# sunshinnnn/DSMnet

Measured on AMD Instinct MI355X. Metric: stereo pairs/sec forward, PSMNet D=192 384×1280, at 1/2/4/8 MI355X, higher is better.
Workload: dtype f32

## Files before the change

dsmnet_amd/csrc/deconv_zs.hpp:

```cpp
#pragma once


template <int PM> struct DzsCfg {
  static constexpr int NP = Prec<PM>::NP, NPW = Prec<PM>::NPW;
  static constexpr int THREADS = 512, NSTAGE = 256;
  static constexpr int TY = 2, IY = TY + 1, IX = 33;
  static constexpr int NV = IY * IX;
  static constexpr int NPF = (NV * 8 + NSTAGE - 1) / NSTAGE;
  static constexpr int NVP = 32 * NPF;
  static constexpr int ROW = NVP * 16;
  static constexpr int IMG = NP * 4 * ROW;
  static constexpr int XPL = 2 * TY * 64 * 8 * 16;
  static constexpr int LDS = 2 * IMG + 2 * XPL;
  static constexpr int NSTEP = 27;
#ifndef DSM_DZS_DEPTH
#define DSM_DZS_DEPTH 4
#endif
  static constexpr int DEPTH = DSM_DZS_DEPTH;
  static_assert(DEPTH == 2 || DEPTH == 4, "the staging loop is unrolled four times");
  static constexpr int WRING = 9, WAHEAD = 8;
  static_assert(NSTEP % WRING == 0 && WAHEAD < WRING, "weight ring");
  static_assert(LDS <= 160 * 1024, "LDS");
};

template <int PM>
__global__ __launch_bounds__(512, 1) void deconv_zs_kernel(ConvParams p) {
  using C = DzsCfg<PM>;
  using T = ZsTerms<PM>;
  using frag = typename Prec<PM>::frag;
  constexpr int NP = C::NP, NPW = C::NPW, TY = C::TY, IX = C::IX, NV = C::NV, NPF = C::NPF, ROW = C::ROW,
                IMG = C::IMG, XPL = C::XPL, NSTEP = C::NSTEP, WRING = C::WRING, WAHEAD = C::WAHEAD;
  extern __shared__ __attribute__((aligned(16))) unsigned char lds_raw[];
  const int tid = threadIdx.x, lane = tid & 63, wave = tid >> 6;
  const bool staging = wave >= 4;
  const int w4 = wave & 3;
  const int ncg = p.Cin >> 5;
  const int NTP = p.Cout >> 5;
  const int MD = (p.Do + 1) >> 1;

  const int G = gridDim.x, id = blockIdx.x;
  const int logical = (G & 7) == 0 ? (id & 7) * (G >> 3) + (id >> 3) : id;
  const long nunits = (long)p.ntiles * MD;
  const long u_begin = nunits * logical / G, u_end = nunits * (logical + 1) / G;
  if (u_begin >= u_end) return;

  const SplitScale ss = split_scale<PM>(p.x_amax, p.w_amax);
  const float sx = ss.sx, so = ss.out;
  unsigned char* const xch = lds_raw + 2 * IMG;
  float am = 0.f;

  struct It { long u; int col, m0, m1, zhi, zi, cg; bool valid; };
  auto open_segment = [&](long u) {
    It q; q.u = u; q.valid = u < u_end;
    if (!q.valid) { q.col = q.m0 = q.m1 = q.zhi = q.zi = q.cg = 0; return q; }
    q.col = (int)(u / MD); q.m0 = (int)(u % MD);
    q.m1 = (int)min((long)MD, (long)q.m0 + (u_end - u));
    q.zhi = 2 * q.m1 - 1 < p.Do ? q.m1 : q.m1 - 1;
    q.zi = q.m0; q.cg = 0;
    return q;
  };
  auto advance = [&](It q) {
    if (++q.cg < ncg) return q;
    q.cg = 0;
    if (++q.zi <= q.zhi) return q;
    return open_segment(q.u + (q.m1 - q.m0));
  };
  auto handover = [&](const It& q) {
    if (!q.valid || q.cg != ncg - 1) return 0u;
    unsigned m = 0;
    if (q.zi - 1 >= q.m0 && q.zi - 1 < q.m1 && 2 * q.zi - 1 < p.Do) m |= 1u;
    if (q.zi >= q.m0 && q.zi < q.m1) m |= 2u;
    return m;
  };

  if (staging) {
    const int stid = tid & 255;
    const unsigned vstride = (unsigned)p.Cin * 4u;
    const unsigned plane_bytes = vstride * (unsigned)p.Hi * (unsigned)p.Wi;
    constexpr unsigned OOBV = 0x80000000u;
    const int sq = 2 * (lane >> 4) + (lane & 1), sv = 8 * w4 + ((lane & 15) >> 1);
    unsigned voff[NPF];
    auto column_offsets = [&](int col) {
      const int t = col / NTP;
      const int y0 = ((t / p.ntx) % p.nty) * TY, x0 = (t % p.ntx) * 32;
#pragma unroll
      for (int k = 0; k < NPF; ++k) {
        const int v = sv + 32 * k;
        const int y = y0 + v / IX, x = x0 + v % IX;
        const bool ok = v < NV && y < p.Hi && x < p.Wi;
        voff[k] = ok ? ((unsigned)y * (unsigned)p.Wi + (unsigned)x) * vstride + 16u * (unsigned)sq : OOBV;
      }
    };
    f32x4 pf[C::DEPTH][NPF];
    auto load_chunk = [&](auto setc, const It& q) {
      constexpr int set = decltype(setc)::value;
      const int b = (q.col / NTP) / (p.ntx * p.nty);
      const bool live = q.valid && q.zi < p.Di;
      const long off = live ? ((long)b * p.Di + q.zi) * (long)plane_bytes + (long)q.cg * 128 : 0;
      const __amdgpu_buffer_rsrc_t rs = make_rsrc(reinterpret_cast<const char*>(p.x) + off, live ? plane_bytes : 0u);
#pragma unroll
      for (int k = 0; k < NPF; ++k) pf[set][k] = buffer_load16(rs, voff[k], 0);
    };
    const int st_off = (lane >> 4) * ROW + sv * 16 + (lane & 1) * 8;
    auto split_chunk = [&](auto setc, unsigned char* wr) {
      constexpr int set = decltype(setc)::value;
#pragma unroll
      for (int k = 0; k < NPF; ++k) {
        unsigned lo[NP], hi[NP];
        split_pair<PM>(pf[set][k].x, pf[set][k].y, sx, lo);
        split_pair<PM>(pf[set][k].z, pf[set][k].w, sx, hi);
#pragma unroll
        for (int q = 0; q < NP; ++q) {
          u32x2 v; v.x = lo[q]; v.y = hi[q];
          *reinterpret_cast<u32x2*>(wr + q * 4 * ROW + 512 * k) = v;
        }
      }
    };
    const int qd = stid & 7, ev = stid >> 3;
    f32x4 sc[2], sh[2];
#pragma unroll
    for (int nb = 0; nb < 2; ++nb) {
      const int c = 32 * (nb < NTP ? nb : 0) + 4 * qd;
#pragma unroll
      for (int e = 0; e < 4; ++e) {
        sc[nb][e] = p.scale ? p.scale[c + e] * so : so;
        sh[nb][e] = p.shift ? p.shift[c + e] : 0.f;
      }
    }
    struct Pend { int col, zi; unsigned m; };
    struct Where { int b, Y0, X0, nb; };
    auto where = [&](int col) {
      Where q;
      const int t = col / NTP;
      q.nb = col - t * NTP;
      q.b = t / (p.ntx * p.nty);
      q.Y0 = 2 * (((t / p.ntx) % p.nty) * TY);
      q.X0 = 2 * ((t % p.ntx) * 32);
      return q;
    };
    f32x4 resq[2][8];
#pragma unroll
    for (int s = 0; s < 2; ++s)
#pragma unroll
      for (int k = 0; k < 8; ++k) resq[s][k] = f32x4{0.f, 0.f, 0.f, 0.f};
    auto vmask_of = [&](const Where& q) {
      unsigned m = 0;
#pragma unroll
      for (int k = 0; k < 8; ++k)
        if (q.Y0 + (k >> 1) < p.Ho && q.X0 + ev + 32 * (k & 1) < p.Wo) m |= 1u << k;
      return m;
    };
    auto load_res = [&](const Pend& e) __attribute__((always_inline)) {
      if (!e.m || !p.res) return;
      const Where q = where(e.col);
      const unsigned vm = vmask_of(q);
#pragma unroll
      for (int s = 0; s < 2; ++s) {
        if (!((e.m >> s) & 1u)) continue;
        const float* const rb = p.res + ((((long)q.b * p.Dr + 2 * e.zi - 1 + s) * p.Hr + q.Y0) * p.Wr + q.X0 + ev) * p.Cout +
                                32 * q.nb + 4 * qd;
#pragma unroll
        for (int k = 0; k < 8; ++k)
          if ((vm >> k) & 1u)
            resq[s][k] = *reinterpret_cast<const f32x4*>(rb + ((k >> 1) * p.Wr + 32 * (k & 1)) * p.Cout);
      }
    };
    const float lo2 = p.relu == 2 ? 0.f : -__builtin_huge_valf(), lo1 = p.relu == 1 ? 0.f : -__builtin_huge_valf();
    auto vmax = [](f32x4 v, float lo) {
      v.x = fmaxf(v.x, lo); v.y = fmaxf(v.y, lo); v.z = fmaxf(v.z, lo); v.w = fmaxf(v.w, lo);
      return v;
    };
    auto epilogue = [&](const Pend& e) __attribute__((always_inline)) {
      if (!e.m) return;
      const Where q = where(e.col);
      const unsigned vm = vmask_of(q);
      const f32x4 s_ = q.nb ? sc[1] : sc[0], h_ = q.nb ? sh[1] : sh[0];
#pragma unroll
      for (int s = 0; s < 2; ++s) {
        if (!((e.m >> s) & 1u)) continue;
        f32x4 v[8];
#pragma unroll
        for (int k = 0; k < 8; ++k) {
          const int oy = k >> 1, ox = ev + 32 * (k & 1);
          v[k] = *reinterpret_cast<const f32x4*>(xch + s * XPL + ((oy * 64 + ox) * 8 + (qd ^ ((ox >> 1) & 7))) * 16);
        }
        float* const yb = p.y + ((((long)q.b * p.Do + 2 * e.zi - 1 + s) * p.Ho + q.Y0) * p.Wo + q.X0 + ev) * p.Cout +
                          32 * q.nb + 4 * qd;
#pragma unroll
        for (int k = 0; k < 8; ++k) {
          if (!((vm >> k) & 1u)) continue;
          f32x4 o = vmax(v[k] * s_ + h_, lo2);
          if (p.res) o += resq[s][k];
          o = vmax(o, lo1);
          *reinterpret_cast<f32x4*>(yb + ((k >> 1) * p.Wo + 32 * (k & 1)) * p.Cout) = o;
          track_amax(am, o);
        }
      }
    };

    constexpr int D = C::DEPTH;
    It c0 = open_segment(u_begin);
    It lead = c0;
    column_offsets(c0.col);
    load_chunk(std::integral_constant<int, 0>{}, lead);
    split_chunk(std::integral_constant<int, 0>{}, lds_raw + st_off);
    static_for<1, D>([&](auto dc) {
      const It nl = advance(lead);
      if (nl.valid && nl.col != lead.col) column_offsets(nl.col);
      lead = nl;
      load_chunk(dc, lead);
    });
    It c1 = advance(c0);
    Pend pend = {0, 0, 0u};
    load_res(Pend{c0.col, c0.zi, handover(c0)});
    __syncthreads();
    auto iteration = [&](auto pc) {
      constexpr int P = decltype(pc)::value;
      const It nl = advance(lead);
      if (nl.valid && nl.col != lead.col) column_offsets(nl.col);
      lead = nl;
      load_chunk(std::integral_constant<int, P % D>{}, lead);
      if (c1.valid) split_chunk(std::integral_constant<int, (P + 1) % D>{}, lds_raw + ((P + 1) & 1) * IMG + st_off);
      epilogue(pend);
      pend = Pend{c0.col, c0.zi, handover(c0)};
      load_res(Pend{c1.col, c1.zi, handover(c1)});
      __syncthreads();
      c0 = c1; c1 = advance(c1);
      return !c0.valid;
    };
    while (true) {
      if (iteration(std::integral_constant<int, 0>{})) break;
      if (iteration(std::integral_constant<int, 1>{})) break;
      if (iteration(std::integral_constant<int, 2>{})) break;
      if (iteration(std::integral_constant<int, 3>{})) break;
    }
    epilogue(pend);
  } else {
    const int j = lane & 15, kg = lane >> 4;
    const int ah = w4 >> 1, xh = w4 & 1;
    const unsigned tstride = (unsigned)NTP * (NPW * 1024);
    const __amdgpu_buffer_rsrc_t wrsrc = make_rsrc(p.w, p.wbytes);
    const unsigned wlane = (unsigned)(kg >> 1) * 27u * tstride + (unsigned)(32 * (kg & 1) + 16 * ah + j) * 16u;
    auto wbase_of = [&](const It& q) {
      return (unsigned)q.cg * 54u * tstride + (unsigned)(q.col % NTP) * (NPW * 1024);
    };
    const int rd_off = kg * ROW + (16 * xh + j) * 16;
    f32x4 acc[3][4][TY];
    frag xq[2][TY][NP];
    frag wq[WRING][NP];
    auto zero_set = [&](auto sc_) {
      constexpr int s = decltype(sc_)::value;
#pragma unroll
      for (int c = 0; c < 4; ++c)
#pragma unroll
        for (int r = 0; r < TY; ++r) acc[s][c][r] = f32x4{0.f, 0.f, 0.f, 0.f};
    };
    auto wload = [&](auto sc_, unsigned wb) {
      constexpr int s = decltype(sc_)::value;
      constexpr int tap = (s % 3) * 9 + dc_tap9(s / 3);
#pragma unroll
      for (int q = 0; q < NP; ++q)
        wq[s % WRING][q] = __builtin_bit_cast(frag, buffer_load16(wrsrc, wlane, wb + (unsigned)tap * tstride + q * 1024));
    };
    auto xload = [&](auto oc, const unsigned char* rd) {
      constexpr int o = decltype(oc)::value, iy = o >> 1, ix = o & 1;
#pragma unroll
      for (int r = 0; r < TY; ++r)
#pragma unroll
        for (int q = 0; q < NP; ++q)
          xq[o & 1][r][q] = *reinterpret_cast<const frag*>(rd + q * 4 * ROW + ((r + iy) * IX + ix) * 16);
    };
    auto zmask_of = [&](const It& q) {
      unsigned m = 0;
      if (q.zi >= q.m0 && q.zi < q.m1) m |= 6u;
      if (q.zi - 1 >= q.m0 && q.zi - 1 < q.m1 && q.zi < p.Di && 2 * q.zi - 1 < p.Do) m |= 1u;
      return m;
    };
    It cur = open_segment(u_begin);
    static_for<0, 3>([&](auto s) { zero_set(s); });
    static_for<0, WAHEAD>([&](auto sc_) { wload(sc_, wbase_of(cur)); });
    int i = 0;
    __syncthreads();
    while (true) {
      const unsigned char* const rd = lds_raw + (i & 1) * IMG + rd_off;
      const It nxt = advance(cur);
      const unsigned wcur = wbase_of(cur);
      const unsigned wnext = nxt.valid ? wbase_of(nxt) : 0u;
      const unsigned mask = zmask_of(cur);
      xload(std::integral_constant<int, 0>{}, rd);
      __builtin_amdgcn_sched_barrier(0);
      static_for<0, NSTEP>([&](auto sc_) {
        constexpr int s = decltype(sc_)::value;
        constexpr int jp = s / 3, kz = s % 3;
        constexpr DcPair pr = dc_pair(jp);
        constexpr bool fresh = kz == 0 && (jp == 0 || jp == 4 || jp == 6 || jp == 8);
        if constexpr (s + WAHEAD < NSTEP) wload(std::integral_constant<int, s + WAHEAD>{}, wcur);
        else wload(std::integral_constant<int, s + WAHEAD - NSTEP>{}, wnext);
        if constexpr (fresh && pr.o + 1 < 4) xload(std::integral_constant<int, pr.o + 1>{}, rd);
        __builtin_amdgcn_sched_barrier(0);
        if ((mask >> kz) & 1u) {
          static_for<0, T::N>([&](auto tc) {
            constexpr int t = decltype(tc)::value;
            static_for<0, TY>([&](auto rc) {
              constexpr int r = decltype(rc)::value;
              acc[kz][pr.c][r] = zs_mfma<PM>(wq[s % WRING][T::w[t]], xq[pr.o & 1][r][T::x[t]], acc[kz][pr.c][r]);
            });
          });
        }
        __builtin_amdgcn_sched_barrier(0);
      });
      if (cur.cg == ncg - 1) {
        const unsigned m = handover(cur);
#pragma unroll
        for (int s = 0; s < 2; ++s) {
          if (!((m >> s) & 1u)) continue;
#pragma unroll
          for (int c = 0; c < 4; ++c)
#pragma unroll
            for (int r = 0; r < TY; ++r) {
              const int oy = 2 * r + (c >> 1), ox = 2 * (16 * xh + j) + (c & 1);
              const int unit = (oy * 64 + ox) * 8 + ((4 * ah + kg) ^ (j & 7));
              *reinterpret_cast<f32x4*>(xch + s * XPL + unit * 16) = acc[s][c][r];
            }
        }
#pragma unroll
        for (int c = 0; c < 4; ++c)
#pragma unroll
          for (int r = 0; r < TY; ++r) acc[0][c][r] = acc[2][c][r];
        zero_set(std::integral_constant<int, 1>{});
        zero_set(std::integral_constant<int, 2>{});
      }
      __syncthreads();
      cur = nxt; ++i;
      if (!cur.valid) break;
    }
  }
  publish_amax<8>(p.y_amax, am, reinterpret_cast<float*>(lds_raw));
}

template <int PM>
int run_deconv_zs(ConvParams p, hipStream_t s) {
  using C = DzsCfg<PM>;
  DSM_REQUIRE(p.Cin % 64 == 0 && (p.Cout == 32 || p.Cout == 64) && 4l * p.Hi * p.Wi * p.Cin < 0x7fffffffl,
              DSM_ERR_UNSUPPORTED);
  p.ntx = dsm_cdiv(p.Wi, 32); p.nty = dsm_cdiv(p.Hi, C::TY);
  const long ncol = (long)p.B * p.nty * p.ntx * (p.Cout / 32);
  DSM_REQUIRE(ncol * p.Di < (1L << 30), DSM_ERR_UNSUPPORTED);
  p.ntiles = (int)ncol;
  const long nunits = ncol * ((p.Do + 1) / 2);
  DSM_REQUIRE(dsm_allow_lds<deconv_zs_kernel<PM>>(C::LDS) == DSM_OK, DSM_ERR_LAUNCH);
  int blocks = p.force_blocks ? p.force_blocks : 256;
  if ((long)blocks > nunits) blocks = (int)nunits;
  hipLaunchKernelGGL(deconv_zs_kernel<PM>, dim3(blocks), dim3(C::THREADS), C::LDS, s, p);
  return dsm_launch_status();
}
```

Before: 207.1.

## Use buffer-descriptor predicated stores and residual loads in the deconv epilogue

Adds a default branch-free epilogue path for the staging waves. Residual loads and output stores go through raw buffer resources built per row, whose byte range is clipped to the valid extent. Out-of-bounds lanes are dropped or zero-filled by hardware rather than by per-element mask branches, and the amax update is masked arithmetically. The epilogue and residual prefetch now alternate between even and odd pipeline iterations instead of both running every iteration. The cost is extra descriptor-building arithmetic, and the result depends on that new cadence matching how columns are produced.

```diff
diff --git a/dsmnet_amd/csrc/deconv_zs.hpp b/dsmnet_amd/csrc/deconv_zs.hpp
--- a/dsmnet_amd/csrc/deconv_zs.hpp
+++ b/dsmnet_amd/csrc/deconv_zs.hpp
@@ -15,6 +15,9 @@
   static constexpr int NSTEP = 27;
 #ifndef DSM_DZS_DEPTH
 #define DSM_DZS_DEPTH 4
+#endif
+#ifndef DSM_DZS_BRANCHY
+#define DSM_DZS_BRANCHY 0
 #endif
   static constexpr int DEPTH = DSM_DZS_DEPTH;
   static_assert(DEPTH == 2 || DEPTH == 4, "the staging loop is unrolled four times");
@@ -138,6 +141,7 @@
       q.X0 = 2 * ((t % p.ntx) * 32);
       return q;
     };
+#if DSM_DZS_BRANCHY
     f32x4 resq[2][8];
 #pragma unroll
     for (int s = 0; s < 2; ++s)
@@ -165,11 +169,13 @@
             resq[s][k] = *reinterpret_cast<const f32x4*>(rb + ((k >> 1) * p.Wr + 32 * (k & 1)) * p.Cout);
       }
     };
+#endif
     const float lo2 = p.relu == 2 ? 0.f : -__builtin_huge_valf(), lo1 = p.relu == 1 ? 0.f : -__builtin_huge_valf();
     auto vmax = [](f32x4 v, float lo) {
       v.x = fmaxf(v.x, lo); v.y = fmaxf(v.y, lo); v.z = fmaxf(v.z, lo); v.w = fmaxf(v.w, lo);
       return v;
     };
+#if DSM_DZS_BRANCHY
     auto epilogue = [&](const Pend& e) __attribute__((always_inline)) {
       if (!e.m) return;
       const Where q = where(e.col);
@@ -197,6 +203,60 @@
         }
       }
     };
+#else
+    auto row_rsrc = [&](const float* base, int Dn, int Hn, int Wn, const Where& q, int z, int oy, bool on) {
+      const bool ok = on && q.Y0 + oy < p.Ho;
+      const long row = ((((long)q.b * Dn + z) * Hn + q.Y0 + oy) * Wn + q.X0) * p.Cout + 32 * q.nb;
+      const long left = ((long)p.Wo - q.X0) * p.Cout * 4 - 128 * q.nb;
+      return make_rsrc(base + (ok ? row : 0l), ok && left > 0 ? (unsigned)left : 0u);
+    };
+    const unsigned eoff[2] = {(unsigned)ev * (unsigned)p.Cout * 4u + 16u * (unsigned)qd,
+                              (unsigned)(ev + 32) * (unsigned)p.Cout * 4u + 16u * (unsigned)qd};
+    typedef unsigned raw16 __attribute__((ext_vector_type(4)));
+    f32x4 resq[2][8];
+#pragma unroll
+    for (int s = 0; s < 2; ++s)
+#pragma unroll
+      for (int k = 0; k < 8; ++k) resq[s][k] = f32x4{0.f, 0.f, 0.f, 0.f};
+    const bool has_res = p.res != nullptr;
+    auto load_res = [&](const Pend& e) __attribute__((always_inline)) {
+      const Where q = where(e.col);
+#pragma unroll
+      for (int s = 0; s < 2; ++s) {
+        const bool on = has_res && ((e.m >> s) & 1u);
+#pragma unroll
+        for (int k = 0; k < 8; ++k)
+          resq[s][k] = buffer_load16(row_rsrc(p.res, p.Dr, p.Hr, p.Wr, q, 2 * e.zi - 1 + s, k >> 1, on), eoff[k & 1], 0);
+      }
+    };
+    auto xch_read = [&](int s, int k) {
+      const int oy = k >> 1, ox = ev + 32 * (k & 1);
+      return *reinterpret_cast<const f32x4*>(xch + s * XPL + ((oy * 64 + ox) * 8 + (qd ^ ((ox >> 1) & 7))) * 16);
+    };
+    auto epilogue = [&](const Pend& e) __attribute__((always_inline)) {
+      const Where q = where(e.col);
+      const f32x4 s_ = q.nb ? sc[1] : sc[0], h_ = q.nb ? sh[1] : sh[0];
+      const int xlim = p.Wo - q.X0 - ev;
+#pragma unroll
+      for (int s = 0; s < 2; ++s) {
+        const bool on = (e.m >> s) & 1u;
+        f32x4 v[8];
+#pragma unroll
+        for (int k = 0; k < 8; ++k) v[k] = xch_read(s, k);
+#pragma unroll
+        for (int k = 0; k < 8; ++k) {
+          f32x4 o = vmax(v[k] * s_ + h_, lo2);
+          if (has_res) o += resq[s][k];
+          o = vmax(o, lo1);
+          __builtin_amdgcn_raw_buffer_store_b128(__builtin_bit_cast(raw16, o),
+                                                 row_rsrc(p.y, p.Do, p.Ho, p.Wo, q, 2 * e.zi - 1 + s, k >> 1, on),
+                                                 (int)eoff[k & 1], 0, 0);
+          const bool inside = on && q.Y0 + (k >> 1) < p.Ho && 32 * (k & 1) < xlim;
+          am = fmaxf(am, inside ? quad_amax(o) : 0.f);
+        }
+      }
+    };
+#endif
 
     constexpr int D = C::DEPTH;
     It c0 = open_segment(u_begin);
@@ -212,6 +272,7 @@
     });
     It c1 = advance(c0);
     Pend pend = {0, 0, 0u};
+#if DSM_DZS_BRANCHY
     load_res(Pend{c0.col, c0.zi, handover(c0)});
     __syncthreads();
     auto iteration = [&](auto pc) {
@@ -235,6 +296,30 @@
       if (iteration(std::integral_constant<int, 3>{})) break;
     }
     epilogue(pend);
+#else
+    __syncthreads();
+    auto iteration = [&](auto pc) {
+      constexpr int P = decltype(pc)::value;
+      const It nl = advance(lead);
+      if (nl.valid && nl.col != lead.col) column_offsets(nl.col);
+      lead = nl;
+      load_chunk(std::integral_constant<int, P % D>{}, lead);
+      if (c1.valid) split_chunk(std::integral_constant<int, (P + 1) % D>{}, lds_raw + ((P + 1) & 1) * IMG + st_off);
+      if constexpr (P % 2 == 0) epilogue(pend);
+      pend = Pend{c0.col, c0.zi, handover(c0)};
+      if constexpr (P % 2 == 1) load_res(pend);
+      __syncthreads();
+      c0 = c1; c1 = advance(c1);
+      return !c0.valid;
+    };
+    while (true) {
+      if (iteration(std::integral_constant<int, 0>{})) break;
+      if (iteration(std::integral_constant<int, 1>{})) break;
+      if (iteration(std::integral_constant<int, 2>{})) break;
+      if (iteration(std::integral_constant<int, 3>{})) break;
+    }
+    epilogue(pend);
+#endif
   } else {
     const int j = lane & 15, kg = lane >> 4;
     const int ah = w4 >> 1, xh = w4 & 1;
```

New measurement: 207.7, median of 6. About the same (+0.3%).
